# iAmGiG/WaveletTransforms

Hardware: AMD Instinct MI355X
Metric: weight-coeffs/s for L5 bior3.3 DWT+thresh+IDWT; achieved HBM GB/s vs peak (higher is better)
Workload: dtype f32; 1 GPU; resnet18_conv_state_dict; config=cfg2, wavelet=bior3.3, level=5, weights_this_rank=11166912, coeffs_this_rank=11166912, tensors=20, graph_steps=10, parallelism=single, transform=2-D over (kh, kw) (reference)

## Files before the change

### include/wtprune.h

```cpp
#ifndef WTPRUNE_H
#define WTPRUNE_H

#include <stddef.h>
#include <stdint.h>

#ifdef __cplusplus
extern "C" {
#endif

typedef struct ihipStream_t* wtp_stream_t;

#define WTP_MAX_DIMS 8
#define WTP_ABI_VERSION 1

#define WTP_OK 0
#define WTP_EBADWAVELET (-1)
#define WTP_EBADLEVEL (-2)
#define WTP_EBADPCT (-3)
#define WTP_EEMPTY (-4)
#define WTP_ECROP (-5)
#define WTP_EARG (-6)
#define WTP_EWORKSPACE (-7)
#define WTP_EHIP (-8)

// ... 53 lines not shown
#define WTP_ABS_PATH_TINY 1
#define WTP_ABS_PATH_CHAIN 2
size_t wtp_abs_workspace_size(const wtp_tensor* tensors, int ntensors, int wavelet_id, int level);
int wtp_prune_abs_f32(const wtp_tensor* tensors, int ntensors, int wavelet_id, int level, double threshold,
                      void* workspace, size_t workspace_bytes, wtp_abs_result* results_dev, wtp_stream_t stream);

int wtp_threshold_f32(const float* in, float* out, int64_t n, double pct, void* workspace,
                      size_t workspace_bytes, wtp_result* result_dev, wtp_stream_t stream);

size_t wtp_dwt_workspace_size(int64_t B, int64_t H, int64_t W, int level);
int wtp_wavedec2_f32(const float* in, float* packed, int64_t B, int64_t H, int64_t W, int wavelet_id,
                     int level, void* workspace, size_t workspace_bytes, wtp_stream_t stream);
int wtp_waverec2_f32(const float* packed, float* out, int64_t B, int64_t H, int64_t W, int wavelet_id,
                     int level, const float* thr32_dev, void* workspace, size_t workspace_bytes,
                     wtp_stream_t stream);

int wtp_synth_f32(float* out, int64_t n, uint64_t seed, uint32_t tensor_id, int e, wtp_stream_t stream);

size_t wtp_min_prune_workspace_size(const wtp_tensor* tensors, int ntensors, double fraction);
int wtp_min_prune_f32(const wtp_tensor* tensors, int ntensors, double fraction, void* workspace,
                      size_t workspace_bytes, wtp_result* results_dev, wtp_stream_t stream);

int wtp_random_prune_f32(const wtp_tensor* tensors, int ntensors, const int64_t* prune_counts, uint64_t seed,
                         wtp_result* results_dev, wtp_stream_t stream);

int wtp_count_small_f32(const float* x, int64_t n, float thr, unsigned long long* count_dev, wtp_stream_t stream);

int wtp_set_stage_events(void* const* events, int n);

int wtp_set_resident(int mode);
int wtp_resident_capacity(void);
unsigned wtp_set_resident_timeout_us(unsigned us);
#define WTP_PATH_FAULT 99
int wtp_set_pipeline(int mode);
int wtp_set_fused_select(int mode);
int wtp_set_interior(int mode);
#define WTP_PATH_SMALL 4
int wtp_set_kernel_stamps(unsigned long long* stamps_dev);

const char* wtp_last_error(void);
int wtp_last_error_tensor(void);

#ifdef __cplusplus
}
#endif
#endif
```

### wavelettransforms_amd/_native.py

```python
import ctypes
import os

import torch

HERE = os.path.dirname(os.path.abspath(__file__))
LIB_PATH = os.environ.get("WTP_LIB_PATH") or os.path.join(HERE, "_lib", "libwtprune.so")
MAX_DIMS = 8

WTP_OK = 0
WTP_EBADWAVELET = -1
WTP_EBADLEVEL = -2
WTP_EBADPCT = -3
WTP_EEMPTY = -4
WTP_ECROP = -5
WTP_EARG = -6
WTP_EWORKSPACE = -7
WTP_EHIP = -8


class WtpTensor(ctypes.Structure):
    _fields_ = [("in_", ctypes.c_void_p), ("out", ctypes.c_void_p), ("ndim", ctypes.c_int32),
                ("reserved", ctypes.c_int32), ("shape", ctypes.c_int64 * MAX_DIMS)]


# ... 31 lines not shown
        sigs = {
            "wtp_abi_version": ([], i32),
            "wtp_wavelet_count": ([], i32),
            "wtp_wavelet_name": ([i32], ctypes.c_char_p),
            "wtp_wavelet_id": ([ctypes.c_char_p], i32),
            "wtp_dec_len": ([i32], i32),
            "wtp_max_level": ([i64, i32], i32),
            "wtp_packed_shape": ([i64, i64, i32, ctypes.POINTER(i64), ctypes.POINTER(i64)], i32),
            "wtp_workspace_size": ([tp, i32, i32, i32], sz),
            "wtp_workspace_init": ([vp, sz, vp], i32),
            "wtp_prune_f32": ([tp, i32, i32, i32, f64, vp, sz, vp, vp], i32),
            "wtp_prune_layers_f32": ([tp, i32, i32, i32, f64, vp, sz, vp, vp], i32),
            "wtp_workspace_size_ex": ([tp, i32, i32, i32, i32], sz),
            "wtp_prune_ex_f32": ([tp, i32, i32, i32, f64, i32, vp, sz, vp, vp], i32),
            "wtp_abs_workspace_size": ([tp, i32, i32, i32], sz),
            "wtp_prune_abs_f32": ([tp, i32, i32, i32, f64, vp, sz, vp, vp], i32),
            "wtp_threshold_f32": ([vp, vp, i64, f64, vp, sz, vp, vp], i32),
            "wtp_dwt_workspace_size": ([i64, i64, i64, i32], sz),
            "wtp_wavedec2_f32": ([vp, vp, i64, i64, i64, i32, i32, vp, sz, vp], i32),
            "wtp_waverec2_f32": ([vp, vp, i64, i64, i64, i32, i32, vp, vp, sz, vp], i32),
            "wtp_synth_f32": ([vp, i64, ctypes.c_uint64, ctypes.c_uint32, i32, vp], i32),
            "wtp_set_stage_events": ([ctypes.POINTER(ctypes.c_void_p), i32], i32),
            "wtp_min_prune_workspace_size": ([tp, i32, f64], sz),
            "wtp_min_prune_f32": ([tp, i32, f64, vp, sz, vp, vp], i32),
            "wtp_random_prune_f32": ([tp, i32, ctypes.POINTER(i64), ctypes.c_uint64, vp, vp], i32),
            "wtp_count_small_f32": ([vp, i64, ctypes.c_float, vp, vp], i32),
            "wtp_set_resident": ([i32], i32),
            "wtp_set_pipeline": ([i32], i32),
            "wtp_set_fused_select": ([i32], i32),
            "wtp_set_interior": ([i32], i32),
            "wtp_resident_capacity": ([], i32),
            "wtp_set_resident_timeout_us": ([ctypes.c_uint], ctypes.c_uint),
            "wtp_set_kernel_stamps": ([vp], i32),
            "wtp_last_error": ([], ctypes.c_char_p),
            "wtp_last_error_tensor": ([], i32),
        }
        missing = {}
        for name, (args, ret) in sigs.items():
            if os.environ.get("WTP_LIB_PATH") and not hasattr(L, name):
                missing[name] = _missing_entry(name)
                continue
            fn = getattr(L, name)
            fn.argtypes = args
            fn.restype = ret
        if L.wtp_abi_version() != 1:
            raise NativeLibraryMissing("libwtprune.so ABI version mismatch")
        _lib = _LabLib(L, missing) if missing else L
    return _lib


def _missing_entry(name):
    def call(*_a, **_k):
        raise NativeLibraryMissing("%s (WTP_LIB_PATH) has no entry point %s: it was built from an older "
                                   "revision" % (LIB_PATH, name))
    return call


class _LabLib:

    def __init__(self, L, missing):
        self._L, self._missing = L, missing

    def __getattr__(self, name):
        if name in self._missing:
            return self._missing[name]
        return getattr(self._L, name)
# ... 13 lines not shown
```

### wavelettransforms_amd/csrc/api.hip

```cpp
#include <algorithm>
#include <atomic>
#include <cmath>
#include <cstdarg>
#include <cstdio>
#include <cstring>
#include <map>
#include <mutex>
#include <string>
#include <vector>

#include "wtp_internal.h"
#include "small_geom.h"
#include "wt_filters.inc"
#include "wt_perm.h"

using namespace wtp;

namespace {

thread_local std::string g_err;
thread_local int g_err_tensor = -1;
thread_local hipEvent_t g_stage_ev[8];
thread_local int g_stage_n = 0;
std::atomic<int> g_resident{1};
// ... 531 lines not shown
int wtp_packed_shape(int64_t H, int64_t W, int level, int64_t* rows, int64_t* cols) {
    if (level < 0 || level > 32 || !rows || !cols) return fail(WTP_EARG, -1, "bad packed-shape request");
    wt_level_geom g;
    wt_geom(H, W, level, &g);
    *rows = g.PR;
    *cols = g.PC;
    return WTP_OK;
}
const char* wtp_last_error(void) { return g_err.c_str(); }
int wtp_set_stage_events(void* const* events, int n) {
    if (n < 0 || n > 8 || (n > 0 && !events)) return fail(WTP_EARG, -1, "bad stage events");
    for (int i = 0; i < 8; ++i) g_stage_ev[i] = (i < n) ? (hipEvent_t)events[i] : nullptr;
    g_stage_n = n;
    return WTP_OK;
}
int wtp_last_error_tensor(void) { return g_err_tensor; }
int wtp_set_resident(int mode) {
    if (mode < 0 || mode > 1) return fail(WTP_EARG, -1, "bad resident mode %d", mode);
    const int prev = g_resident.exchange(mode);
    return prev;
}
int wtp_resident_capacity(void) { return resident_capacity(); }
int wtp_set_interior(int mode) { return fb_set_interior(mode); }

int wtp_set_pipeline(int mode) {
    if (mode < 0 || mode > 1) return fail(WTP_EARG, -1, "bad pipeline mode %d", mode);
    return g_pipeline.exchange(mode);
}
int wtp_set_fused_select(int mode) {
    if (mode < 0 || mode > 1) return fail(WTP_EARG, -1, "bad fused-select mode %d", mode);
    return g_fused.exchange(mode);
}
unsigned wtp_set_resident_timeout_us(unsigned us) { return set_resident_timeout_us(us); }
int wtp_set_kernel_stamps(unsigned long long* stamps_dev) {
    set_kernel_stamps(stamps_dev);
    return WTP_OK;
}

size_t wtp_workspace_size(const wtp_tensor* tensors, int ntensors, int wavelet_id, int level) {
    if (ntensors < 0 || (ntensors > 0 && !tensors)) return 0;
    std::vector<TPlan> ps, pl;
    if (plan_tensors(tensors, ntensors, wavelet_id, level, 50.0, false, ps, true) != WTP_OK) return 0;
    if (plan_tensors(tensors, ntensors, wavelet_id, level, 50.0, false, pl, false) != WTP_OK) return 0;
    const Taps tp = (wavelet_id >= 0 && wavelet_id < WT_NUM_WAVELETS) ? make_taps(wavelet_id) : Taps{};
    return std::max(make_layout(ps, tp).total, make_layout(pl, tp).total);
}

int wtp_workspace_init(void* ws, size_t bytes, wtp_stream_t stream) {
    if (!ws && bytes) return fail(WTP_EARG, -1, "null workspace");
    if (bytes && hipMemsetAsync(ws, 0, bytes, (hipStream_t)stream) != hipSuccess)
        return fail(WTP_EHIP, -1, "hipMemsetAsync failed");
    return WTP_OK;
}

struct SidePipe {
    hipStream_t side = nullptr;
    std::vector<hipEvent_t> ev;
};
std::mutex g_pipe_mu;
std::map<std::pair<int, hipStream_t>, SidePipe> g_pipes;
SidePipe* side_pipe(hipStream_t s, int nev) {
    int dev = 0, sdev = 0;
    if (hipGetDevice(&dev) != hipSuccess) return nullptr;
    if (hipStreamGetDevice(s, &sdev) != hipSuccess || sdev != dev) return nullptr;
    std::lock_guard<std::mutex> lk(g_pipe_mu);
    SidePipe& sp = g_pipes[{dev, s}];
// ... 710 lines not shown
```

### wavelettransforms_amd/csrc/kernels.hip

```cpp
#include "wtp_internal.h"
#include "wt_synth.h"
#include "wt_perm.h"

#include <atomic>
#include <cstdlib>

#pragma clang fp contract(off)

namespace wtp {

__device__ __forceinline__ uint32_t abs_key(float x) { return __float_as_uint(x) & 0x7FFFFFFFu; }

template <bool COH, class T>
__device__ __forceinline__ T ldc(const T* p) {
    if constexpr (COH) return __hip_atomic_load(const_cast<T*>(p), __ATOMIC_RELAXED, __HIP_MEMORY_SCOPE_AGENT);
    else return *p;
}
template <class T>
__device__ __forceinline__ void stc(T* p, T v) {
    __hip_atomic_store(p, v, __ATOMIC_RELAXED, __HIP_MEMORY_SCOPE_AGENT);
}
__device__ __forceinline__ __amdgpu_buffer_rsrc_t region_rsrc(const uint32_t* p, int words) {
    const uint64_t a = reinterpret_cast<uint64_t>(p);
    const uint32_t lo = __builtin_amdgcn_readfirstlane((uint32_t)a), hi = __builtin_amdgcn_readfirstlane((uint32_t)(a >> 32));
// ... 1364 lines not shown
                                          wtp_result* __restrict__ res, int64_t base, int len, bool al) {
    constexpr int CT = RES_THREADS, IT = RES_IT;
    const int tid = threadIdx.x;
    float* qo = sd.out + base;
    auto fin = [&](float xv) { return (fabsf(xv) < thr) ? 0.0f : xv; };
    if (FULL) {
        float4* q4 = reinterpret_cast<float4*>(qo);
#pragma unroll
        for (int it = 0; it < IT; ++it) {
            typedef float f4v __attribute__((ext_vector_type(4)));
            const f4v yv = {fin(v[it].x), fin(v[it].y), fin(v[it].z), fin(v[it].w)};
            __builtin_nontemporal_store(yv, reinterpret_cast<f4v*>(q4 + it * CT + tid));
        }
    } else {
        const __amdgpu_buffer_rsrc_t rr = ragged_rsrc(qo, len);
#pragma unroll
        for (int it = 0; it < IT; ++it) {
            const float4 y = make_float4(fin(v[it].x), fin(v[it].y), fin(v[it].z), fin(v[it].w));
            store4_tail(y, qo, rr, it * CT + tid, len, al);
        }
    }
    if (thr != thr) {
        uint32_t z = 0;
#pragma unroll
        for (int it = 0; it < IT; ++it)
#pragma unroll
            for (int c = 0; c < 4; ++c) z += f4_get(v[it], c) == 0.0f;
        const unsigned long long tot = block_sum_u64<CT>(z) - (unsigned long long)(RES_CHUNK - len);
        if (tid == 0 && tot) atomicAdd((unsigned long long*)&res[sd.res].zero_count, tot);
    }
    WTP_RPROBE(7);
}

template <bool FULL>
__device__ __forceinline__ void res_body(const SegTable& t, const SegDesc& sd, SelHeader* __restrict__ head, uint32_t qv,
                                         uint32_t* __restrict__ cand, wtp_result* __restrict__ res,
                                         float* __restrict__ thr_out, int64_t base, int len, uint32_t* raw,
                                         uint32_t* lsub, uint32_t (*wred)[8], uint32_t* wstage, bool sel) {
    constexpr int CT = RES_THREADS, IT = RES_IT, NW = CT / 64;
    uint32_t q = 0;
    const bool first = base == 0 && !sel;
    const int tid = threadIdx.x, wv = tid >> 6, lane = tid & 63;
    const uint64_t tmo = t.res_timeout;
    WTP_RPROBE(0);
    WTP_RTAG(sd.flags);
    __shared__ uint32_t s_win[3];
    __shared__ uint32_t s_sync;
    __shared__ uint32_t s_pubn;
    __shared__ uint32_t s_arr;
    float4 v[IT];
    uint32_t arr1 = 0;
    {
        uint32_t ks[RES_SPL];
        const int64_t n = sd.n;
        const bool exact = n <= RES_MS;
        const int m = exact ? (int)n : RES_MS;
        if (wv < RES_SW) {
            const uint32_t sl = (uint32_t)sd.res_step_fx, shi = (uint32_t)(sd.res_step_fx >> 32);
#pragma unroll
            for (int j = 0; j < RES_SPL; ++j) {
                const int i = j * (64 * RES_SW) + tid;
                const uint32_t g = (uint32_t)i / SAMPLE_GROUP;
                const int pos = exact ? min(i, (int)n - 1)
                                      : (int)(__umulhi(g, sl) + g * shi) + (i % SAMPLE_GROUP);
                ks[j] = __float_as_uint(sd.data[pos]);
            }
// ... 208 lines not shown
        if (!ovf && !sel) {
            const __amdgpu_buffer_rsrc_t prs = region_rsrc(pub, RES_PUB_WORDS);
            if (tid < RES_NSUB / 4) {
                const int b = 4 * tid;
                st16_sc1(prs, b, make_uint4(b ? pos[b - 1] : 0u, pos[b], pos[b + 1], pos[b + 2]));
            } else if (tid == RES_NSUB / 4) {
                stc(pub + RES_NSUB, pos[RES_NSUB - 1]);
            }
            const uint32_t nin = pos[RES_NSUB - 1];
            for (uint32_t i4 = tid; 4 * i4 < nin; i4 += ST)
                st16_sc1(prs, RES_PUB_KEYS + 4 * i4, *reinterpret_cast<const uint4*>(srt + 4 * i4));
        }
        asm volatile("s_waitcnt vmcnt(0)" ::: "memory");
        if (!sel && lane == 0 && atomicAdd(&s_pubn, 1u) == (uint32_t)(NW - 2)) atomicAdd(b2, 1u);
        if (wv == NW - 2 && lane == 0) {
            const uint32_t sh8 = blockIdx.x & (NSHARD - 1);
            const uint32_t nsh = (gridDim.x - sh8 + NSHARD - 1) / NSHARD;
            const uint32_t nact = min((uint32_t)NSHARD, gridDim.x);
            if (s_arr == nsh - 1u && atomicAdd(&bar->arrive[0][16], 1u) == nact - 1u) stc(&head->parity, q + 1u);
        }
    }
    __syncthreads();
    WTP_RPROBE(11);
    uint64_t* gr = reinterpret_cast<uint64_t*>(&st->thr_gr);
    if (!s_ok1) {
        if (tid == 0) {
            atomicMax(&res[sd.res].path, (int32_t)MODE_FAULT);
            if (sel) atomicCAS(reinterpret_cast<unsigned long long*>(gr), 0ull, (unsigned long long)RES_GR_FAULT << 32);
        }
        return;
    }
    WTP_RPROBE(5);
    if (remote && !sel) {
        __shared__ unsigned long long s_gr;
        if (wv == NW - 1 && lane == 0) {
            const uint64_t t0 = wall_ticks();
            unsigned long long x;
            while (true) {
                x = ldc<true>(reinterpret_cast<const unsigned long long*>(gr));
                if (x) break;
                if (wall_ticks() - t0 >= tmo) {
                    const unsigned long long f = (unsigned long long)RES_GR_FAULT << 32;
                    const unsigned long long o = atomicCAS(reinterpret_cast<unsigned long long*>(gr), 0ull, f);
                    x = o ? o : f;
                    break;
                }
                __builtin_amdgcn_s_sleep(2);
            }
            s_gr = x;
        }
        __syncthreads();
        const unsigned long long g = s_gr;
        const uint32_t tag = (uint32_t)(g >> 32);
        if (tag & RES_GR_FAULT) {
            if (tid == 0) atomicMax(&res[sd.res].path, (int32_t)MODE_FAULT);
            return;
        }
        const float thr = __uint_as_float((uint32_t)g);
        WTP_RPROBE(6);
        res_final<FULL>(v, thr, sd, res, base, len, al);
        return;
    }
    __shared__ uint32_t s_wtot[NW], s_b2;
    __shared__ int s_bk[2];
    __shared__ uint32_t s_bef[2], s_bn[2];
    if (!solo) {
        if (tid == 0) {
            unsigned long long x[NSHARD];
#pragma unroll
            for (int i = 0; i < NSHARD; ++i) x[i] = ldc<true>(st->below + i);
            unsigned long long sum = 0;
#pragma unroll
            for (int i = 0; i < NSHARD; ++i) sum += x[i];
            s_cnt[0] = sum;
        } else if (tid == 2) {
            uint32_t x[NSHARD];
#pragma unroll
            for (int i = 0; i < NSHARD; ++i) x[i] = ldc<true>(st->maxkey + i);
            uint32_t mm = 0;
#pragma unroll
            for (int i = 0; i < NSHARD; ++i) mm = max(mm, x[i]);
            s_mk = mm;
        } else if (tid == 3) {
            s_ovf = ldc<true>(&st->overflow);
        } else if (tid == 4) {
// ... 21 lines not shown
        if (r < sbelow) return 0;
        r -= sbelow;
        if (r < (int64_t)ninside) { *j = r; return 2; }
        return 0;
    };
    int64_t ja = 0, jb = 0;
    const int ca = classify(r0, &ja), cb = classify(r1, &jb);
#pragma unroll
    for (int i = 0; i < 2; ++i) {
        const int64_t j = i == 0 ? ja : jb;
        if ((i == 0 ? ca : cb) == 2 && j >= (int64_t)excl && j < (int64_t)(excl + cs)) {
            uint32_t e = excl;
            int b = BPT * tid;
#pragma unroll
            for (int u = 0; u < BPT - 1; ++u) {
                const bool past = j >= (int64_t)(e + cb8[u]) && b == BPT * tid + u;
                e += past ? cb8[u] : 0u;
                b += past ? 1 : 0;
            }
            s_bk[i] = b;
            s_bef[i] = e;
            s_bn[i] = cb8[b - BPT * tid];
        }
    }
    __syncthreads();
    WTP_PROBE(2);
    bool full = ca == 0 || cb == 0 || s_ovf != 0;
    int path = MODE_WINDOW;
    uint32_t ka = kl, kb = kl;
    uint32_t before = 0;
    int m = 0;
    uint32_t* stage = raw;
    const uint32_t* sel_keys = stage;
    if (!full && (ca == 2 || cb == 2)) {
        const int ba = ca == 2 ? s_bk[0] : s_bk[1], bb = cb == 2 ? s_bk[1] : s_bk[0];
        before = ca == 2 ? s_bef[0] : s_bef[1];
        const uint32_t nlo = ca == 2 ? s_bn[0] : s_bn[1], nhi = (bb != ba) ? s_bn[1] : 0u;
        m = (int)(nlo + nhi);
        if (solo) {
            sel_keys = srt + (ba ? pos[ba - 1] : 0u);
            const uint32_t lo = (uint32_t)((uint64_t)kl + ((uint64_t)ba << sh));
            const uint32_t hi = (uint32_t)min((uint64_t)kh, (uint64_t)kl + ((uint64_t)(bb + 1) << sh) - 1);
            uint32_t xa = kl, xb = kl;
            select_in_range<CT>([&](int64_t i) { return sel_keys[i]; }, [](uint32_t) { return true; }, (int64_t)m, lo,
                                hi, ja - (int64_t)before, jb - (int64_t)before, ca == 2, cb == 2, &xa, &xb);
            ka = ca == 2 ? xa : kl;
            kb = cb == 2 ? xb : kl;
            path = MODE_CAND;
        } else if (m > RES_SEL_MAX) {
            full = true;
        } else {
            WTP_PROBE(3);
            const uint32_t b2v = s_b2;
            if (!(b2v >= nwg && !(b2v & RES_POISON)) && !res_wait(b2, nwg, tmo)) {
                if (tid == 0) {
                    atomicMax(&res[sd.res].path, (int32_t)MODE_FAULT);
                    if (sel) atomicCAS(reinterpret_cast<unsigned long long*>(gr), 0ull, (unsigned long long)RES_GR_FAULT << 32);
                }
                return;
            }
            WTP_PROBE(4);
            const int wb = sd.blk_begin;
            __shared__ uint32_t s_so[RES_MAX_WG], s_ob[RES_MAX_WG];
            __shared__ uint32_t s_tot;
            if (wv == 0) {
                constexpr int WPL = RES_MAX_WG / 64;
                uint32_t ob[WPL], oe[WPL];
#pragma unroll
                for (int u = 0; u < WPL; ++u) {
                    const int w = lane + 64 * u;
                    const uint32_t* pw = cand + (int64_t)(wb + min(w, (int)nwg - 1)) * RES_PUB_WORDS;
                    ob[u] = ldc<true>(pw + ba);
                    oe[u] = ldc<true>(pw + bb + 1);
                }
                uint32_t base = 0;
#pragma unroll
                for (int u = 0; u < WPL; ++u) {
                    const int w = lane + 64 * u;
                    const uint32_t cw = w < (int)nwg ? oe[u] - ob[u] : 0u;
                    const uint32_t inc = wave_scan_u32(cw);
                    if (w < (int)nwg) { s_so[w] = base + inc - cw; s_ob[w] = ob[u]; }
                    base += __builtin_amdgcn_readlane(inc, 63);
                }
                if (lane == 0) s_tot = base;
// ... 15 lines not shown
                                      ((uint32_t)i - s_so[lo_w]));
                }
#pragma unroll
                for (int u = 0; u < 2; ++u)
                    if (tid + u * CT < m) stage[tid + u * CT] = kv[u];
                __syncthreads();
                WTP_PROBE(5);
                const uint32_t lo = (uint32_t)((uint64_t)kl + ((uint64_t)ba << sh));
                const uint32_t hi = (uint32_t)min((uint64_t)kh, (uint64_t)kl + ((uint64_t)(bb + 1) << sh) - 1);
                uint32_t xa = kl, xb = kl;
                select_in_range<CT>([&](int64_t i) { return stage[i]; }, [](uint32_t) { return true; }, (int64_t)m,
                                    lo, hi, ja - (int64_t)before, jb - (int64_t)before, ca == 2, cb == 2, &xa, &xb);
                ka = ca == 2 ? xa : kl;
                kb = cb == 2 ? xb : kl;
                path = MODE_CAND;
            }
        }
    }
    WTP_PROBE(6);
    if (full) {
        const float* x = sd.data;
        select_in_range<CT>([&](int64_t i) { return abs_key(x[i]); }, [](uint32_t) { return true; }, sd.n, 0u,
                            0xFFFFFFFFu, r0, r1, true, true, &ka, &kb);
        path = MODE_FULL;
    }
    const float fa = __uint_as_float(ka), fb = __uint_as_float(kb);
    const float diff = fb - fa;
    const double g = sd.gamma;
    double thr64 = (g >= 0.5) ? (double)fb - (double)diff * (1.0 - g) : (double)fa + (double)diff * g;
    if (mk > 0x7F800000u) thr64 = __longlong_as_double(0x7FF8000000000000ll);
    const float thr = (float)thr64;
    const bool nan = thr != thr;
    if (sel && tid == 0) {
        const uint32_t tag = RES_GR_OK | (path == MODE_FULL ? RES_GR_ALL : 0u);
        const unsigned long long gv = ((unsigned long long)tag << 32) | __float_as_uint(thr);
        if (atomicCAS(reinterpret_cast<unsigned long long*>(gr), 0ull, gv) != 0ull)
            atomicMax(&res[sd.res].path, (int32_t)MODE_FAULT);
    }
    WTP_RPROBE(6);
    if (first || sel) {
        unsigned long long zc = 0;
        if (!nan) {
            const uint32_t tk = thr > 0.0f ? __float_as_uint(thr) : 1u;
            if (path == MODE_FULL) {
                zc = (unsigned long long)block_count_below<CT>([&](int64_t i) { return abs_key(sd.data[i]); }, sd.n, tk);
            } else {
                uint32_t c = 0;
                if (path == MODE_CAND)
                    for (int i = tid; i < m; i += CT) c += sel_keys[i] < tk;
                const unsigned long long sc = block_sum_u64<CT>(c);
                zc = (unsigned long long)sbelow +
                     (path == MODE_CAND ? (unsigned long long)before : 0ull) + sc;
            }
        }
        if (tid == 0) {
            thr_out[sd.res] = thr;
            wtp_result& r = res[sd.res];
            r.numel = sd.numel;
            r.coeff_numel = sd.n;
            if (zc) atomicAdd((unsigned long long*)&r.zero_count, zc);
            r.thr64 = thr64;
            r.thr32_bits = __float_as_uint(thr);
            r.max_abs_bits = mk;
            r.eff_level = sd.eff_level;
            atomicMax(&r.path, path);
        }
    }
// ... 446 lines not shown
    if (masked) {
        hipLaunchKernelGGL(k_mask_select, dim3(t.nblk), dim3(STREAM_THREADS), 0, s, t, head, cand, res, thr_out);
        return;
    }
    SegTable d = t;
    for (int i = 0; i < t.nseg; ++i) d.s[i].blk_begin = d.blk_begin[i] = i;
    d.nblk = t.nseg;
    hipLaunchKernelGGL(k_mask_select, dim3(d.nblk), dim3(STREAM_THREADS), 0, s, d, head, cand, res, thr_out);
}
void launch_mask_inplace(const SegTable& t, const wtp_result* res, const float* thr, hipStream_t s) {
    hipLaunchKernelGGL(k_mask_inplace, dim3(t.nblk), dim3(STREAM_THREADS), 0, s, t, res, thr);
}
int resident_capacity() {
    static std::atomic<int> cache[16];
    int dev = 0;
    if (hipGetDevice(&dev) != hipSuccess || dev < 0) return 0;
    if (dev < 16) {
        const int c = cache[dev].load(std::memory_order_relaxed);
        if (c) return c > 0 ? c : 0;
    }
    int per = 0, cus = 0;
    int cap = -1;
    if (hipOccupancyMaxActiveBlocksPerMultiprocessor(&per, k_resident, RES_THREADS, 0) == hipSuccess &&
        hipDeviceGetAttribute(&cus, hipDeviceAttributeMultiprocessorCount, dev) == hipSuccess && per >= 1 && cus > 0)
        cap = cus;
    (void)hipGetLastError();
    if (dev < 16) cache[dev].store(cap, std::memory_order_relaxed);
    return cap > 0 ? cap : 0;
}
static std::atomic<uint32_t> g_res_timeout_us{RES_TIMEOUT_DEFAULT_US};
uint32_t set_resident_timeout_us(uint32_t us) { return g_res_timeout_us.exchange(std::min(us, RES_TIMEOUT_MAX_US)); }
static std::atomic<unsigned long long*> g_stamps{nullptr};
void set_kernel_stamps(unsigned long long* dev) { g_stamps.store(dev); }
uint32_t resident_timeout_us() { return g_res_timeout_us.load(std::memory_order_relaxed); }
unsigned long long* kernel_stamps() { return g_stamps.load(std::memory_order_relaxed); }
void launch_resident(const SegTable& t0, SelHeader* head, uint32_t* cand, wtp_result* res, float* thr_out,
                     hipStream_t s) {
    SegTable t = t0;
    t.res_timeout = g_res_timeout_us.load(std::memory_order_relaxed) * 100u;
    t.stamps = g_stamps.load(std::memory_order_relaxed);
    int nshared = 0;
    for (int i = 0; i < t.nseg; ++i) nshared += t.s[i].n > RES_CHUNK;
    t.nsel = 0;
    if (nshared > 0 && t.nblk + nshared <= RES_MAX_WG && t.nblk + nshared <= resident_capacity())
        for (int i = 0; i < t.nseg; ++i)
            if (t.s[i].n > RES_CHUNK) t.sel_seg[t.nsel++] = i;
    hipLaunchKernelGGL(k_resident, dim3(t.nblk + t.nsel), dim3(RES_THREADS), 0, s, t, head, cand, res, thr_out);
}
void launch_dwt_cols(const float* in, int64_t B, int64_t R, int64_t C, const Taps& tp, float* L, float* H,
                     hipStream_t s) {
    hipLaunchKernelGGL(k_dwt_cols, dim3(grid_for(B * ((R + 1) / 2) * C)), dim3(DWT_THREADS), 0, s, in, B, R, C, tp,
                       L, H);
}
void launch_dwt_rows(const float* L, const float* H, int64_t B, int64_t Ro, int64_t C, const Taps& tp, float* anext,
                     float* P, int64_t PR, int64_t PC, int64_t offR, int64_t offC, int last, hipStream_t s) {
    hipLaunchKernelGGL(k_dwt_rows, dim3(grid_for(B * Ro * ((C + 1) / 2))), dim3(DWT_THREADS), 0, s, L, H, B, Ro, C,
                       tp, anext, P, PR, PC, offR, offC, last);
}
void launch_idwt_rows(const float* a, int64_t a_bs, int64_t lda, int a_from_P, const float* P, int64_t PR, int64_t PC,
                      int64_t offR, int64_t offC, int64_t B, int64_t R, int64_t C, const Taps& tp, const float* thr,
                      float* lo, float* hi, hipStream_t s) {
    hipLaunchKernelGGL(k_idwt_rows, dim3(grid_for(B * R * 2 * C)), dim3(DWT_THREADS), 0, s, a, a_bs, lda, a_from_P,
                       P, PR, PC, offR, offC, B, R, C, tp, thr, lo, hi);
}
void launch_idwt_cols(const float* lo, const float* hi, int64_t B, int64_t R, int64_t C, const Taps& tp, float* y,
                      int64_t outH, int64_t outW, unsigned long long* zero_count, hipStream_t s) {
    hipLaunchKernelGGL(k_idwt_cols, dim3(grid_for(B * outH * outW)), dim3(DWT_THREADS), 0, s, lo, hi, B, R, 2 * C, tp,
                       y, outH, outW, zero_count);
}
void launch_dwt1_level(const float* x, int64_t N, const Taps& tp, float* a, float* d, hipStream_t s) {
    hipLaunchKernelGGL(k_dwt1_level, dim3(grid_for((N + 1) / 2)), dim3(DWT_THREADS), 0, s, x, N, tp, a, d);
}
void launch_idwt1_level(const float* a, int a_thr, const float* d, int64_t N, const Taps& tp, const float* thr,
// ... 26 lines not shown
```

### wavelettransforms_amd/csrc/wtp_internal.h

```cpp
#ifndef WTP_INTERNAL_H
#define WTP_INTERNAL_H

#include <hip/hip_runtime.h>
#include <stdint.h>

#include "../../include/wtprune.h"
#include "wt_dwt_core.h"
#include "wt_abs_core.h"

#pragma clang fp contract(off)

namespace wtp {

constexpr int M_SAMPLE = 4096;
constexpr int M_SAMPLE_WIN = 65536;
constexpr int SAMPLE_GROUP = 16;
constexpr int NSUB_MAX = 1024;
constexpr int RES_NSUB_LOG2 = 10;
constexpr int RES_NSUB = 1 << RES_NSUB_LOG2;
constexpr int BUCKET_MAX = 8192;
constexpr int BUCKET_MAX_DWT = 1 << 16;
constexpr int WIN_EXP = 32;
constexpr int MANT_BITS = 7;
constexpr uint32_t WIN_E0 = 101;
constexpr int NB = 3 + (WIN_EXP << MANT_BITS);
constexpr int BIN_ZERO = 0, BIN_UNDER = 1, BIN_OVER = NB - 1;

__host__ __device__ __forceinline__ int key_bin(uint32_t key) {
    if (key == 0) return BIN_ZERO;
    const uint32_t e = key >> 23;
    if (e < WIN_E0) return BIN_UNDER;
    if (e >= WIN_E0 + WIN_EXP) return BIN_OVER;
    return 2 + (int)(((e - WIN_E0) << MANT_BITS) | ((key >> (23 - MANT_BITS)) & ((1u << MANT_BITS) - 1)));
}
__host__ __device__ __forceinline__ uint32_t bin_lo_key(int b) {
    if (b <= BIN_ZERO) return 0u;
// ... 19 lines not shown
    SEG_KZERO = 8,
    SEG_LATE = 16,
    SEG_FUSED = 32,
};

struct SegDesc {
    const float* data;
    float* out;
    int64_t n;
    int64_t r0;
    double gamma;
    int64_t numel;
    int32_t blk_begin;
    int32_t slot;
    int32_t res;
    int32_t flags;
    int32_t eff_level;
    int32_t above;
    int64_t cand_off;
    int64_t cap;
    int32_t nsub_log2;
    int32_t bucket_cap;
    uint64_t res_step_fx;
};
__host__ __device__ inline const uint32_t* seg_fsl(const SegDesc& sd) { return reinterpret_cast<const uint32_t*>(sd.out); }
__host__ __device__ inline int32_t seg_fsl_n(const SegDesc& sd) { return (int32_t)sd.res_step_fx; }

struct SegTable {
    int32_t nseg;
    int32_t nblk;
    int32_t nsel;
    int32_t retry;
    uint32_t res_timeout;
    int32_t pad2;
    unsigned long long* stamps;
    int32_t blk_begin[SEG_PER_LAUNCH];
    int32_t sel_seg[SEG_PER_LAUNCH];
    SegDesc s[SEG_PER_LAUNCH];
};
static_assert(sizeof(SegTable) <= 4096, "k_resident's kernel argument");


constexpr int NSHARD = 8;
struct alignas(128) SelState {
    unsigned long long below[NSHARD];
    unsigned long long eq_lo[NSHARD];
    unsigned long long eq_hi[NSHARD];
    unsigned long long seg_bar[NSHARD];
    uint32_t maxkey[NSHARD];
    uint32_t overflow;
    uint32_t pad0a;
    unsigned long long thr_gr;
    uint32_t pad0[20];
    uint32_t kl, kh;
    uint32_t shift;
    int32_t mode;
    float thr32;
    uint32_t key_a, key_b;
    uint32_t pad1[25];
    uint32_t sub[RES_NSUB];
};
static_assert(sizeof(SelState) % 128 == 0 && sizeof(SelState) == 512 + 4 * RES_NSUB, "SelState layout");

struct alignas(128) SelHeader {
    uint32_t parity;
    uint32_t done;
    uint32_t pad[30];
};
struct alignas(128) BarState {
    uint32_t arrive[NSHARD][32];
};
constexpr size_t SEL_REGION = SEG_PER_LAUNCH * sizeof(SelState) + sizeof(BarState);
__host__ __device__ inline SelState* sel_region(void* head, uint32_t q) {
    return reinterpret_cast<SelState*>(reinterpret_cast<char*>(head) + sizeof(SelHeader) + (size_t)(q & 1u) * SEL_REGION);
}
__host__ __device__ inline BarState* bar_region(void* head, uint32_t q) {
    return reinterpret_cast<BarState*>(reinterpret_cast<char*>(sel_region(head, q)) + SEG_PER_LAUNCH * sizeof(SelState));
}

enum SelMode : int32_t { MODE_CAND = 1, MODE_WINDOW = 2, MODE_FULL = 3, MODE_RETRY = 5, MODE_RETRIED = 8,
                         MODE_FAULT = 99 };

constexpr int FSL_WORDS = 64;
constexpr int FSL_KEYS = FSL_WORDS - 1;
constexpr int FWIN_PS = 128;
constexpr int FWIN_NP = 4;
constexpr int FWIN_THREADS = 1024;
constexpr int FSC_THREADS = 256;
constexpr int FSC_SLOTS = 64 * (FSC_THREADS / 64);
constexpr int FWIN_F_MAX = 18;
static_assert(FWIN_NP * FWIN_PS * FWIN_PS == M_SAMPLE_WIN, "k_fwin's sample is k_window's");
struct alignas(256) FslHeader {
    uint32_t kl, kh, shift;
    uint32_t pad0[29];
    unsigned long long be[NSHARD];
    uint32_t maxkey[NSHARD];
    uint32_t overflow;
    uint32_t pad1[7];
    uint32_t pad2[32];
};
// ... 28 lines not shown
void launch_window(const SegTable& t, SelHeader* head, hipStream_t s, const wtp_result* res = nullptr);
void launch_fused_retry(const SegTable& t, SelHeader* head, uint32_t* cand, wtp_result* res, float* thr_out,
                        hipStream_t s);
void launch_collect(const SegTable& t, SelHeader* head, uint32_t* cand, wtp_result* res, hipStream_t s);
void launch_mask_select(const SegTable& t, SelHeader* head, const uint32_t* cand, wtp_result* res, float* thr_out,
                        hipStream_t s);
void launch_mask_inplace(const SegTable& t, const wtp_result* res, const float* thr, hipStream_t s);
constexpr int RES_THREADS = 512;
constexpr int RES_IT = 24;
constexpr int RES_CHUNK = RES_THREADS * RES_IT * 4;
constexpr int RES_MS = 4096;
constexpr int RES_SW = 4;
constexpr int RES_SPL = RES_MS / (64 * RES_SW);
static_assert(RES_SPL + RES_IT <= 63 && RES_SPL * 64 * RES_SW == RES_MS, "k_resident sample geometry");
constexpr int RES_SIGMA_X100 = 400;
constexpr int RES_MAX_WG = 256;
constexpr int RES_LATE_PCT = 60;
constexpr int RES_STG = 32;
constexpr int RES_PUB_KEYS = (RES_NSUB + 1 + 3) / 4 * 4;
constexpr int RES_PUB_WORDS = RES_PUB_KEYS + RES_STG * RES_THREADS;
constexpr int RES_WG_WORDS = RES_PUB_WORDS;
constexpr int RES_SEL_MAX = 1024;
constexpr uint32_t RES_TIMEOUT_DEFAULT_US = 2000;
int resident_capacity();
constexpr uint32_t RES_TIMEOUT_MAX_US = 40000000u;
uint32_t set_resident_timeout_us(uint32_t us);
void set_kernel_stamps(unsigned long long* dev);
uint32_t resident_timeout_us();
unsigned long long* kernel_stamps();
constexpr uint32_t RES_POISON = 0x80000000u;
constexpr uint32_t RES_GR_OK = 1u;
constexpr uint32_t RES_GR_ALL = 2u;
constexpr uint32_t RES_GR_FAULT = 4u;
void launch_resident(const SegTable& t, SelHeader* head, uint32_t* cand, wtp_result* res, float* thr_out,
                     hipStream_t s);
constexpr int SM_MAX_SEG = 4;
constexpr int SM_SEG_WG_MAX = 128;
constexpr int SM_SLOT_WORDS = 64;
constexpr int SM_ARENA = 34 * 1024;
constexpr int SM_F_MAX = 20;
constexpr int SM_LMAX = 10;
constexpr int SM_WIN_WORDS = 480;
constexpr int SM_LINE_MAX = 32767;
struct SmallSeg {
    const float* in;
    float* out;
    float* P;
    int64_t r0;
    double gamma;
    int64_t numel;
    int64_t n;
    int32_t B, L, PR, PC;
    int32_t R[SM_LMAX + 1], C[SM_LMAX + 1], offR[SM_LMAX + 1], offC[SM_LMAX + 1];
    int32_t TR, TC, tilesR, tilesC;
    int32_t wg_begin, nwg, res, above, npad;
    int32_t win_off;
};
struct SmallTaps {
    int32_t F;
    int32_t pad[3];
    float f[4][SM_F_MAX];
};
struct SmallTable {
    int32_t nseg, nblk;
    uint32_t timeout;
    int32_t pad;
// ... 112 lines not shown
```

### wavelettransforms_amd/engine.py

```python
import ctypes
import warnings

import numpy as np
import torch

from . import _native as N

RESULT_DTYPE = np.dtype([("numel", "<i8"), ("zero_count", "<i8"), ("coeff_numel", "<i8"), ("thr64", "<f8"),
                         ("thr32_bits", "<u4"), ("max_abs_bits", "<u4"), ("eff_level", "<i4"), ("path", "<i4")])
assert RESULT_DTYPE.itemsize == N.RESULT_BYTES

_workspaces = {}


def wavelet_id(name):
    return N.lib().wtp_wavelet_id(str(name).encode()) if isinstance(name, str) else -1


def workspace(device, nbytes, stream=None, kind=None):
    device = torch.device(device)
    if device.index is None:
        device = torch.device(device.type, torch.cuda.current_device())
    if stream is None:
        stream = torch.cuda.current_stream(device)
# ... 134 lines not shown
def carried_level(tensors, wavelet, level, flatten=False):
    L = N.lib()
    F = L.wtp_dec_len(wavelet_id(wavelet))
    lvl = int(level)
    for x in tensors:
        if x.dim() >= 2:
            n = x.numel() if flatten else min(x.shape[-2], x.shape[-1])
            lvl = min(lvl, int(L.wtp_max_level(int(n), int(F))))
    return lvl


def fault_mask(results_dev, n):
    host = results_dev.cpu().numpy().view(RESULT_DTYPE)[:n]
    return host["path"] == MODE_FAULT


def decode(results_dev, n):
    host = results_dev.cpu().numpy().view(RESULT_DTYPE)[:n]
    out = []
    if (host["path"] == MODE_FAULT).any():
        raise RuntimeError("wavelettransforms_amd: records of a resident launch that timed out (MODE_FAULT); "
                           "re-run those tensors with no_resident=True (prune() does this itself)")
    for r in host:
        d = {k: r[k].item() for k in RESULT_DTYPE.names}
        d["thr32"] = float(np.array(d["thr32_bits"], np.uint32).view(np.float32))
        d["max_abs"] = np.array(d["max_abs_bits"], np.uint32).view(np.float32)[()]
        d["nonzero"] = d["numel"] - d["zero_count"]
        out.append(d)
    return out


def set_resident(enabled):
    return bool(N.lib().wtp_set_resident(1 if enabled else 0))


def set_pipeline(enabled):
    mode = (1 if enabled else 0) if isinstance(enabled, bool) else int(enabled)
    return int(N.lib().wtp_set_pipeline(mode))


def set_fused_select(enabled):
    return int(N.lib().wtp_set_fused_select(1 if enabled else 0))


def set_interior(enabled):
    mode = (3 if enabled else 0) if isinstance(enabled, bool) else int(enabled)
    return int(N.lib().wtp_set_interior(mode))


def resident_capacity():
    return int(N.lib().wtp_resident_capacity())


def prune(tensors, wavelet, level, pct, outs=None, carry_level=True, flatten=False):
    outs, res = launch(tensors, wavelet, level, pct, outs=outs, carry_level=carry_level, flatten=flatten)
    if res is None:
        return outs, []
    n = len(tensors)
    bad = fault_mask(res, n)
    if bad.any():
        idx = [i for i in range(n) if bad[i]]
        groups = {}
        for i in idx:
            lvl = carried_level(tensors[:i], wavelet, level, flatten) if carry_level else int(level)
            groups.setdefault(lvl, []).append(i)
        merged = res.clone().view(n, N.RESULT_BYTES)
# ... 190 lines not shown
```

Measured before the change: 415.5 billion weight-coeffs/s.

## Publish threshold bounds early so remote workgroups store unambiguous outputs before final threshold

The selecting workgroup now publishes a key-range bound [lo,hi] for the threshold once the candidate bucket is known. Remote workgroups that were waiting on the final threshold poll both words, and when only the bound is available they store every output slot whose values fall entirely outside the bound. They then wait for the final threshold and store only the deferred slots. This overlaps output writes with the selection barrier, at the cost of a second poll loop, extra control flow, and a fallback to a full rewrite if the final threshold lands outside the published bound.

```diff
diff --git a/include/wtprune.h b/include/wtprune.h
--- a/include/wtprune.h
+++ b/include/wtprune.h
@@ -109,6 +109,9 @@
 int wtp_resident_capacity(void);
 unsigned wtp_set_resident_timeout_us(unsigned us);
 #define WTP_PATH_FAULT 99
+int wtp_set_resident_early(int mode);
+int wtp_resident_early_counts(void* workspace, wtp_stream_t stream, unsigned long long* early,
+                              unsigned long long* deferred);
 int wtp_set_pipeline(int mode);
 int wtp_set_fused_select(int mode);
 int wtp_set_interior(int mode);
diff --git a/wavelettransforms_amd/_native.py b/wavelettransforms_amd/_native.py
--- a/wavelettransforms_amd/_native.py
+++ b/wavelettransforms_amd/_native.py
@@ -87,6 +87,9 @@
             "wtp_resident_capacity": ([], i32),
             "wtp_set_resident_timeout_us": ([ctypes.c_uint], ctypes.c_uint),
             "wtp_set_kernel_stamps": ([vp], i32),
+            "wtp_set_resident_early": ([i32], i32),
+            "wtp_resident_early_counts": ([vp, vp, ctypes.POINTER(ctypes.c_ulonglong),
+                                           ctypes.POINTER(ctypes.c_ulonglong)], i32),
             "wtp_last_error": ([], ctypes.c_char_p),
             "wtp_last_error_tensor": ([], i32),
         }
diff --git a/wavelettransforms_amd/csrc/api.hip b/wavelettransforms_amd/csrc/api.hip
--- a/wavelettransforms_amd/csrc/api.hip
+++ b/wavelettransforms_amd/csrc/api.hip
@@ -587,6 +587,22 @@
     return g_fused.exchange(mode);
 }
 unsigned wtp_set_resident_timeout_us(unsigned us) { return set_resident_timeout_us(us); }
+int wtp_set_resident_early(int mode) {
+    if (mode < 0 || mode > 2) return fail(WTP_EARG, -1, "bad resident early-store mode %d", mode);
+    return set_resident_early(mode);
+}
+int wtp_resident_early_counts(void* ws, wtp_stream_t stream, unsigned long long* early, unsigned long long* deferred) {
+    if (!ws || !early || !deferred) return fail(WTP_EARG, -1, "bad early-count request");
+    SelHeader* head = reinterpret_cast<SelHeader*>(ws);
+    uint32_t c[2] = {0u, 0u};
+    hipStream_t s = (hipStream_t)stream;
+    if (hipMemcpyAsync(c, &head->early_ws, sizeof(c), hipMemcpyDeviceToHost, s) != hipSuccess ||
+        hipMemsetAsync(&head->early_ws, 0, sizeof(c), s) != hipSuccess || hipStreamSynchronize(s) != hipSuccess)
+        return fail(WTP_EHIP, -1, "reading the early-store counters failed");
+    *early = c[0];
+    *deferred = c[1];
+    return WTP_OK;
+}
 int wtp_set_kernel_stamps(unsigned long long* stamps_dev) {
     set_kernel_stamps(stamps_dev);
     return WTP_OK;
diff --git a/wavelettransforms_amd/csrc/kernels.hip b/wavelettransforms_amd/csrc/kernels.hip
--- a/wavelettransforms_amd/csrc/kernels.hip
+++ b/wavelettransforms_amd/csrc/kernels.hip
@@ -1420,6 +1420,69 @@
     WTP_RPROBE(7);
 }
 
+
+__device__ __forceinline__ void res_poll_pair(const SelState* st, unsigned long long* thr, unsigned long long* bnd) {
+    typedef uint32_t u4v __attribute__((ext_vector_type(4)));
+    u4v x;
+    const unsigned long long* p = &st->thr_gr;
+    asm volatile("global_load_dwordx4 %0, %1, off sc1\n\ts_waitcnt vmcnt(0)" : "=&v"(x) : "v"(p) : "memory");
+    *thr = ((unsigned long long)x.y << 32) | x.x;
+    *bnd = ((unsigned long long)x.w << 32) | x.z;
+}
+
+template <bool FULL>
+__device__ __forceinline__ void res_store_slot(const float4& y, float* qo, __amdgpu_buffer_rsrc_t rr, int it, int len,
+                                               bool al) {
+    const int j = it * RES_THREADS + (int)threadIdx.x;
+    if (FULL) {
+        typedef float f4v __attribute__((ext_vector_type(4)));
+        const f4v yv = {y.x, y.y, y.z, y.w};
+        __builtin_nontemporal_store(yv, reinterpret_cast<f4v*>(qo) + j);
+    } else {
+        store4_tail(y, qo, rr, j, len, al);
+    }
+}
+
+template <bool FULL, bool STORE>
+__device__ __forceinline__ uint32_t res_early_stores(const float4 (&v)[RES_IT], uint32_t lo, uint32_t hi,
+                                                     const SegDesc& sd, int64_t base, int len, bool al) {
+    float* qo = sd.out + base;
+    const __amdgpu_buffer_rsrc_t rr = ragged_rsrc(qo, FULL ? 0 : len);
+    const uint32_t w = hi - lo;
+    uint32_t pend = 0;
+#pragma unroll
+    for (int it = 0; it < RES_IT; ++it) {
+        uint32_t k4[4];
+#pragma unroll
+        for (int c = 0; c < 4; ++c) k4[c] = abs_key(f4_get(v[it], c));
+        const bool in = (k4[0] - lo <= w) | (k4[1] - lo <= w) | (k4[2] - lo <= w) | (k4[3] - lo <= w);
+        if (__ballot(in) != 0ull) {
+            pend |= 1u << it;
+        } else if (STORE) {
+            const float4 y = make_float4(k4[0] < lo ? 0.0f : v[it].x, k4[1] < lo ? 0.0f : v[it].y,
+                                         k4[2] < lo ? 0.0f : v[it].z, k4[3] < lo ? 0.0f : v[it].w);
+            res_store_slot<FULL>(y, qo, rr, it, len, al);
+        }
+    }
+    return pend;
+}
+
+template <bool FULL>
+__device__ __forceinline__ void res_pending_stores(const float4 (&v)[RES_IT], uint32_t pend, float thr,
+                                                   const SegDesc& sd, int64_t base, int len, bool al) {
+    float* qo = sd.out + base;
+    const __amdgpu_buffer_rsrc_t rr = ragged_rsrc(qo, FULL ? 0 : len);
+    auto fin = [&](float xv) { return (fabsf(xv) < thr) ? 0.0f : xv; };
+    pend = __builtin_amdgcn_readfirstlane(pend);
+#pragma unroll
+    for (int it = 0; it < RES_IT; ++it)
+        if (pend & (1u << it)) {
+            const float4 y = make_float4(fin(v[it].x), fin(v[it].y), fin(v[it].z), fin(v[it].w));
+            res_store_slot<FULL>(y, qo, rr, it, len, al);
+        }
+    WTP_RPROBE(7);
+}
+
 template <bool FULL>
 __device__ __forceinline__ void res_body(const SegTable& t, const SegDesc& sd, SelHeader* __restrict__ head, uint32_t qv,
                                          uint32_t* __restrict__ cand, wtp_result* __restrict__ res,
@@ -1694,13 +1757,16 @@
     }
     WTP_RPROBE(5);
     if (remote && !sel) {
-        __shared__ unsigned long long s_gr;
+        __shared__ unsigned long long s_gr, s_bnd;
+        const bool early = t.res_early != 0;
         if (wv == NW - 1 && lane == 0) {
             const uint64_t t0 = wall_ticks();
-            unsigned long long x;
+            unsigned long long x, b = 0ull;
             while (true) {
-                x = ldc<true>(reinterpret_cast<const unsigned long long*>(gr));
+                if (early) res_poll_pair(st, &x, &b);
+                else x = ldc<true>(reinterpret_cast<const unsigned long long*>(gr));
                 if (x) break;
+                if (b) break;
                 if (wall_ticks() - t0 >= tmo) {
                     const unsigned long long f = (unsigned long long)RES_GR_FAULT << 32;
                     const unsigned long long o = atomicCAS(reinterpret_cast<unsigned long long*>(gr), 0ull, f);
@@ -1710,9 +1776,57 @@
                 __builtin_amdgcn_s_sleep(2);
             }
             s_gr = x;
+            s_bnd = b;
         }
         __syncthreads();
-        const unsigned long long g = s_gr;
+        unsigned long long g = s_gr;
+        if (g == 0ull) {
+            const unsigned long long bw = s_bnd;
+            const uint32_t lo = (uint32_t)bw, hi = (uint32_t)(bw >> 32) & ~RES_BND_VALID;
+            WTP_RPROBE(20);
+            uint32_t pend;
+            if (wv == NW - 1 && !RES_EARLY_POLL_STORES) pend = res_early_stores<FULL, false>(v, lo, hi, sd, base, len, al);
+            else pend = res_early_stores<FULL, true>(v, lo, hi, sd, base, len, al);
+            WTP_RPROBE(21);
+            if (t.res_early == 2 && lane == 0) {
+                const uint32_t nd = (uint32_t)__builtin_popcount(pend);
+                atomicAdd(&head->early_ws, (uint32_t)IT - nd);
+                if (nd) atomicAdd(&head->defer_ws, nd);
+            }
+            __syncthreads();
+            if (wv == NW - 1 && lane == 0) {
+                const uint64_t t0 = wall_ticks();
+                unsigned long long x;
+                while (true) {
+                    x = ldc<true>(reinterpret_cast<const unsigned long long*>(gr));
+                    if (x) break;
+                    if (wall_ticks() - t0 >= tmo) {
+                        const unsigned long long f = (unsigned long long)RES_GR_FAULT << 32;
+                        const unsigned long long o = atomicCAS(reinterpret_cast<unsigned long long*>(gr), 0ull, f);
+                        x = o ? o : f;
+                        break;
+                    }
+                    __builtin_amdgcn_s_sleep(2);
+                }
+                s_gr = x;
+            }
+            __syncthreads();
+            g = s_gr;
+            const uint32_t tag2 = (uint32_t)(g >> 32);
+            if (tag2 & RES_GR_FAULT) {
+                if (tid == 0) atomicMax(&res[sd.res].path, (int32_t)MODE_FAULT);
+                return;
+            }
+            const float thr2 = __uint_as_float((uint32_t)g);
+            WTP_RPROBE(6);
+            if ((tag2 & RES_GR_ALL) || thr2 != thr2) {
+                res_final<FULL>(v, thr2, sd, res, base, len, al);
+            } else {
+                if (wv == NW - 1 && !RES_EARLY_POLL_STORES) pend = (1u << IT) - 1u;
+                res_pending_stores<FULL>(v, pend, thr2, sd, base, len, al);
+            }
+            return;
+        }
         const uint32_t tag = (uint32_t)(g >> 32);
         if (tag & RES_GR_FAULT) {
             if (tid == 0) atomicMax(&res[sd.res].path, (int32_t)MODE_FAULT);
@@ -1800,6 +1914,8 @@
     int m = 0;
     uint32_t* stage = raw;
     const uint32_t* sel_keys = stage;
+    bool bnd_pub = false;
+    uint32_t blo = 0, bhi = 0;
     if (!full && (ca == 2 || cb == 2)) {
         const int ba = ca == 2 ? s_bk[0] : s_bk[1], bb = cb == 2 ? s_bk[1] : s_bk[0];
         before = ca == 2 ? s_bef[0] : s_bef[1];
@@ -1818,6 +1934,14 @@
         } else if (m > RES_SEL_MAX) {
             full = true;
         } else {
+            if (sel && t.res_early != 0 && ca == 2 && cb == 2 && mk <= 0x7F800000u && sd.out != sd.data && kl > 0u &&
+                kh != 0xFFFFFFFFu) {
+                blo = (uint32_t)((uint64_t)kl + ((uint64_t)ba << sh));
+                bhi = (uint32_t)min((uint64_t)kh, (uint64_t)kl + ((uint64_t)(bb + 1) << sh) - 1);
+                bnd_pub = bhi < 0x7F800000u;
+                if (bnd_pub && tid == 0)
+                    stc(&st->bnd_gr, ((unsigned long long)(bhi | RES_BND_VALID) << 32) | blo);
+            }
             WTP_PROBE(3);
             const uint32_t b2v = s_b2;
             if (!(b2v >= nwg && !(b2v & RES_POISON)) && !res_wait(b2, nwg, tmo)) {
@@ -1899,7 +2023,7 @@
     const float thr = (float)thr64;
     const bool nan = thr != thr;
     if (sel && tid == 0) {
-        const uint32_t tag = RES_GR_OK | (path == MODE_FULL ? RES_GR_ALL : 0u);
+        const uint32_t tag = RES_GR_OK | ((path == MODE_FULL || (bnd_pub && (ka < blo || kb > bhi))) ? RES_GR_ALL : 0u);
         const unsigned long long gv = ((unsigned long long)tag << 32) | __float_as_uint(thr);
         if (atomicCAS(reinterpret_cast<unsigned long long*>(gr), 0ull, gv) != 0ull)
             atomicMax(&res[sd.res].path, (int32_t)MODE_FAULT);
@@ -2412,6 +2536,24 @@
 uint32_t set_resident_timeout_us(uint32_t us) { return g_res_timeout_us.exchange(std::min(us, RES_TIMEOUT_MAX_US)); }
 static std::atomic<unsigned long long*> g_stamps{nullptr};
 void set_kernel_stamps(unsigned long long* dev) { g_stamps.store(dev); }
+static int env_resident_early() {
+    const char* e = getenv("WTP_RESIDENT_EARLY");
+    return (e && e[0] >= '0' && e[0] <= '2' && !e[1]) ? e[0] - '0' : 1;
+}
+static std::atomic<int> g_res_early{-1};
+int resident_early() {
+    int m = g_res_early.load(std::memory_order_relaxed);
+    if (m < 0) {
+        int want = env_resident_early();
+        if (g_res_early.compare_exchange_strong(m, want)) m = want;
+    }
+    return m;
+}
+int set_resident_early(int mode) {
+    const int prev = resident_early();
+    g_res_early.store(mode);
+    return prev;
+}
 uint32_t resident_timeout_us() { return g_res_timeout_us.load(std::memory_order_relaxed); }
 unsigned long long* kernel_stamps() { return g_stamps.load(std::memory_order_relaxed); }
 void launch_resident(const SegTable& t0, SelHeader* head, uint32_t* cand, wtp_result* res, float* thr_out,
@@ -2419,6 +2561,7 @@
     SegTable t = t0;
     t.res_timeout = g_res_timeout_us.load(std::memory_order_relaxed) * 100u;
     t.stamps = g_stamps.load(std::memory_order_relaxed);
+    t.res_early = resident_early();
     int nshared = 0;
     for (int i = 0; i < t.nseg; ++i) nshared += t.s[i].n > RES_CHUNK;
     t.nsel = 0;
diff --git a/wavelettransforms_amd/csrc/wtp_internal.h b/wavelettransforms_amd/csrc/wtp_internal.h
--- a/wavelettransforms_amd/csrc/wtp_internal.h
+++ b/wavelettransforms_amd/csrc/wtp_internal.h
@@ -2,6 +2,7 @@
 #define WTP_INTERNAL_H
 
 #include <hip/hip_runtime.h>
+#include <stddef.h>
 #include <stdint.h>
 
 #include "../../include/wtprune.h"
@@ -87,7 +88,7 @@
     int32_t nsel;
     int32_t retry;
     uint32_t res_timeout;
-    int32_t pad2;
+    int32_t res_early;
     unsigned long long* stamps;
     int32_t blk_begin[SEG_PER_LAUNCH];
     int32_t sel_seg[SEG_PER_LAUNCH];
@@ -104,9 +105,10 @@
     unsigned long long seg_bar[NSHARD];
     uint32_t maxkey[NSHARD];
     uint32_t overflow;
-    uint32_t pad0a;
+    uint32_t pad0a[3];
     unsigned long long thr_gr;
-    uint32_t pad0[20];
+    unsigned long long bnd_gr;
+    uint32_t pad0[16];
     uint32_t kl, kh;
     uint32_t shift;
     int32_t mode;
@@ -116,11 +118,15 @@
     uint32_t sub[RES_NSUB];
 };
 static_assert(sizeof(SelState) % 128 == 0 && sizeof(SelState) == 512 + 4 * RES_NSUB, "SelState layout");
+static_assert(offsetof(SelState, thr_gr) % 16 == 0 && offsetof(SelState, bnd_gr) == offsetof(SelState, thr_gr) + 8 &&
+                  offsetof(SelState, kl) == 384,
+              "SelState granule pair");
 
 struct alignas(128) SelHeader {
     uint32_t parity;
     uint32_t done;
-    uint32_t pad[30];
+    uint32_t early_ws, defer_ws;
+    uint32_t pad[28];
 };
 struct alignas(128) BarState {
     uint32_t arrive[NSHARD][32];
@@ -215,6 +221,10 @@
 constexpr uint32_t RES_GR_OK = 1u;
 constexpr uint32_t RES_GR_ALL = 2u;
 constexpr uint32_t RES_GR_FAULT = 4u;
+constexpr uint32_t RES_BND_VALID = 0x80000000u;
+constexpr bool RES_EARLY_POLL_STORES = true;
+int set_resident_early(int mode);
+int resident_early();
 void launch_resident(const SegTable& t, SelHeader* head, uint32_t* cand, wtp_result* res, float* thr_out,
                      hipStream_t s);
 constexpr int SM_MAX_SEG = 4;
diff --git a/wavelettransforms_amd/engine.py b/wavelettransforms_amd/engine.py
--- a/wavelettransforms_amd/engine.py
+++ b/wavelettransforms_amd/engine.py
@@ -190,6 +190,29 @@
 
 def set_resident(enabled):
     return bool(N.lib().wtp_set_resident(1 if enabled else 0))
+
+
+def set_resident_early(mode):
+    mode = (1 if mode else 0) if isinstance(mode, bool) else int(mode)
+    prev = int(N.lib().wtp_set_resident_early(mode))
+    if prev < 0:
+        raise ValueError(N.last_error())
+    return prev
+
+
+def resident_early_counts(device="cuda", stream=None):
+    device = torch.device(device)
+    if device.index is None:
+        device = torch.device(device.type, torch.cuda.current_device())
+    if stream is None:
+        stream = torch.cuda.current_stream(device)
+    ws = workspace(device, 256, stream)
+    a, b = ctypes.c_ulonglong(0), ctypes.c_ulonglong(0)
+    rc = N.lib().wtp_resident_early_counts(ws.data_ptr(), ctypes.c_void_p(stream.cuda_stream), ctypes.byref(a),
+                                           ctypes.byref(b))
+    if rc != N.WTP_OK:
+        raise RuntimeError("libwtprune: %s (status %d)" % (N.last_error(), rc))
+    return int(a.value), int(b.value)
 
 
 def set_pipeline(enabled):
```

Result: faster. 433.3 billion weight-coeffs/s (median of 6 runs) (+4.3%).
